# big-nacho/patolette

Hardware: AMD Instinct MI355X
Metric: Mpixels/sec quantized (256-color ICtCp + KMeans) at 1 GPU; palette ΔE vs ref (higher is better)
Workload: dtype f64

## Files before the change

patolette_amd/csrc/kmeans.hip:

```cpp
#include "kmeans.h"

namespace pamd {

typedef __attribute__((address_space(1))) const void gvoid_t;
typedef __attribute__((address_space(3))) void lvoid_t;

template <bool W>
__global__ __launch_bounds__(256) void k_km_gather(const double *__restrict__ planar, size_t N, const int *__restrict__ perm,
                                                   size_t nx, KmSamples s) {
    const size_t stride = (size_t)gridDim.x * blockDim.x;
    for (size_t i = (size_t)blockIdx.x * blockDim.x + threadIdx.x; i < nx; i += stride) {
        size_t p = perm ? (size_t)perm[i] : i;
        s.x[i] = (float)planar[p]; s.y[i] = (float)planar[N + p]; s.z[i] = (float)planar[2 * N + p];
        if constexpr (W) s.w[i] = (float)planar[3 * N + p];
    }
}

template <bool W>
__global__ __launch_bounds__(256) void k_km_gather_slice(const double *__restrict__ planar, size_t n_local, const int *__restrict__ perm,
                                                         size_t nx, size_t begin, KmSamples s) {
    const size_t stride = (size_t)gridDim.x * blockDim.x;
    for (size_t i = (size_t)blockIdx.x * blockDim.x + threadIdx.x; i < nx; i += stride) {
        const size_t g = perm ? (size_t)perm[i] : i;
        const bool mine = g >= begin && g - begin < n_local;
// ... 1184 lines not shown
    }
    return acc;
}

template <bool W, int C>
__device__ __forceinline__ float km_chain(const float4 *__restrict__ sorted, size_t lo, size_t hi, float4 (*stage)[64], int lane) {
    return km_chain_over<W, C>([=](const size_t i) { return sorted[lo + i]; }, hi - lo, stage, lane, 0.f);
}

template <int CTRL>
__device__ __forceinline__ double dpp_f64(const double v) {
    const unsigned long long b = (unsigned long long)__double_as_longlong(v);
    const int lo = __builtin_amdgcn_update_dpp(0, (int)(unsigned)b, CTRL, 0xf, 0xf, true);
    const int hi = __builtin_amdgcn_update_dpp(0, (int)(unsigned)(b >> 32), CTRL, 0xf, 0xf, true);
    return __longlong_as_double((long long)(((unsigned long long)(unsigned)hi << 32) | (unsigned)lo));
}
__device__ __forceinline__ double readlane_f64(const double v, const int l) {
    const unsigned long long b = (unsigned long long)__double_as_longlong(v);
    const unsigned lo = (unsigned)__builtin_amdgcn_readlane((int)(unsigned)b, l), hi = (unsigned)__builtin_amdgcn_readlane((int)(unsigned)(b >> 32), l);
    return __longlong_as_double((long long)(((unsigned long long)hi << 32) | lo));
}
__device__ __forceinline__ double wave_sum_dpp(double v) {
    v += dpp_f64<0xB1>(v);
    v += dpp_f64<0x4E>(v);
    v += dpp_f64<0x141>(v);
    v += dpp_f64<0x140>(v);
    return (readlane_f64(v, 0) + readlane_f64(v, 16)) + (readlane_f64(v, 32) + readlane_f64(v, 48));
}

__device__ __forceinline__ bool km_block_exact(const float *blk, const float *wblk, const bool wx, const int q0, const int nq, float &acc, const int lane) {
    const float aa = fabsf(acc);
    if (!(aa >= 1e-30f && aa < 1e30f)) return false;
    int ex;
    (void)frexpf(aa, &ex);
    const double sgn = acc < 0.f ? -1.0 : 1.0;
    const double scale = ldexp(sgn, 24 - ex);
    const double M0 = (double)aa * fabs(scale);
    double tot = 0.0, mag = 0.0, dev = 0.0;
    for (int q = q0; q < q0 + nq; q++) {
        const float4 xv = *reinterpret_cast<const float4 *>(blk + q * 256 + lane * 4);
        float4 wv = make_float4(1.f, 1.f, 1.f, 1.f);
        if (wx) wv = *reinterpret_cast<const float4 *>(wblk + q * 256 + lane * 4);
        const float xs[4] = {xv.x, xv.y, xv.z, xv.w}, ws[4] = {wv.x, wv.y, wv.z, wv.w};
#pragma unroll
        for (int e = 0; e < 4; e++) {
            const double x = (double)xs[e] * (double)ws[e];
            const double t = x * scale;
            const double r = rint(t);
            dev = fmax(dev, fabs(t - r));
            tot += r; mag += fabs(r);
        }
    }
    tot = wave_sum_dpp(tot); mag = wave_sum_dpp(mag);
    const double pp = 0.5 * (tot + mag), nn = 0.5 * (tot - mag);
    if (!__any(dev >= 0.5) && M0 + nn >= 8388609.0 && M0 + pp <= 16777215.0) {
        acc = (float)(ldexp(M0 + tot, ex - 24) * sgn);
        return true;
    }
    return false;
}
__device__ __forceinline__ void km_block_replay(const float *blk, const float *wblk, const bool wx, const unsigned from, const unsigned to, float &acc) {
    for (unsigned base = from; base < to; base += 64) {
        const int cnt = (int)(to - base < 64 ? to - base : 64);
        const float4 *s4 = reinterpret_cast<const float4 *>(blk + base), *w4 = reinterpret_cast<const float4 *>(wblk + base);
        if (cnt == 64) {
            float4 xv[16], wv[16];
#pragma unroll
            for (int q = 0; q < 16; q++) { xv[q] = s4[q]; if (wx) wv[q] = w4[q]; }
            if (wx) {
#pragma unroll
                for (int q = 0; q < 16; q++) {
                    acc = __builtin_fmaf(xv[q].x, wv[q].x, acc); acc = __builtin_fmaf(xv[q].y, wv[q].y, acc);
                    acc = __builtin_fmaf(xv[q].z, wv[q].z, acc); acc = __builtin_fmaf(xv[q].w, wv[q].w, acc);
                }
            } else {
#pragma unroll
                for (int q = 0; q < 16; q++) { acc += xv[q].x; acc += xv[q].y; acc += xv[q].z; acc += xv[q].w; }
            }
        } else {
            for (int q = 0; 4 * q < cnt; q++) {
                const float4 x = s4[q];
                float4 w = make_float4(0, 0, 0, 0);
                if (wx) w = w4[q];
                const float xs[4] = {x.x, x.y, x.z, x.w}, ws[4] = {w.x, w.y, w.z, w.w};
#pragma unroll
                for (int e = 0; e < 4; e++) {
                    if (4 * q + e < cnt) {
                        if (wx) acc = __builtin_fmaf(xs[e], ws[e], acc);
                        else acc += xs[e];
                    }
                }
            }
        }
    }
}
__device__ __forceinline__ void km_block_step(const float *blk, const float *wblk, const bool wx, const unsigned len, float &acc, const int lane) {
    if (km_block_exact(blk, wblk, wx, 0, 4, acc, lane)) return;
    if (len == 1024u) {
        for (int q = 0; q < 4; q++)
            if (!km_block_exact(blk, wblk, wx, q, 1, acc, lane)) km_block_replay(blk, wblk, wx, (unsigned)q * 256u, (unsigned)(q + 1) * 256u, acc);
        return;
    }
    km_block_replay(blk, wblk, wx, 0u, len, acc);
}

template <bool W>
__device__ __forceinline__ float km_chain_coop(const float4 *__restrict__ sorted, size_t lo, size_t hi, float *coop, int lane, int wid) {
    constexpr int K = 16;
    constexpr size_t BS = (size_t)64 * K, SS = 4 * BS;
    const bool wx = W && wid < 3;
    const bool chain = W || wid < 3;
    const float *mine = coop + (size_t)wid * SS, *wts = coop + 3 * SS;
    float acc = 0.f;
    float4 reg[K];
    auto fetch = [&](const size_t p0) {
#pragma unroll
        for (int j = 0; j < K; j++) {
            const size_t i = p0 + (size_t)wid * BS + (size_t)j * 64 + lane;
            reg[j] = make_float4(0, 0, 0, 0);
            if (i < hi) reg[j] = sorted[i];
        }
    };
    fetch(lo);
    for (size_t p0 = lo; p0 < hi; p0 += SS) {
#pragma unroll
        for (int j = 0; j < K; j++) {
            const int o = wid * (int)BS + j * 64 + lane;
            coop[o] = reg[j].x; coop[SS + o] = reg[j].y; coop[2 * SS + o] = reg[j].z; coop[3 * SS + o] = reg[j].w;
        }
        if (p0 + SS < hi) fetch(p0 + SS);
        __syncthreads();
        if (chain) {
            for (int d = 0; d < 4; d++) {
                const size_t pos = p0 + (size_t)d * BS;
                if (pos >= hi) break;
                const size_t bend = pos + BS < hi ? pos + BS : hi;
                const float *blk = mine + d * (int)BS, *wblk = wts + d * (int)BS;
                km_block_step(blk, wblk, wx, (unsigned)(bend - pos), acc, lane);
            }
        }
        __syncthreads();
    }
    return acc;
}

template <bool W>
__device__ __forceinline__ float km_coop_lds(const float *mine, const float *wts, const unsigned n, const bool wx, float acc, const int lane) {
    constexpr unsigned BS = 1024;
    for (unsigned pos = 0; pos < n; pos += BS)
        km_block_step(mine + pos, wts + pos, wx, pos + BS < n ? BS : n - pos, acc, lane);
    return acc;
}

template <bool W, int HS>
__device__ __forceinline__ void km_update_finish(const int kidx, const int k, const unsigned long long nx, const size_t cnt, const float *res,
                                                 int *s_last, float *cent, float *hassign, float4 *c4, unsigned int *ticket, DevMT *mt,
                                                 float *hs_mem = nullptr, unsigned int *flags = nullptr, const bool clean = false) {
    const int lane = threadIdx.x & 63, wid = threadIdx.x >> 6;
    float c0 = res[0], c1 = res[1], c2 = res[2], h = res[3];
    if constexpr (!W) {
        h = cnt < (size_t)16777216 ? (float)cnt : 16777216.0f;
    }
    if (threadIdx.x == 0) {
        if (!clean) {
        if (h != 0.f) { const float norm = 1 / h; c0 *= norm; c1 *= norm; c2 *= norm; }
        __hip_atomic_store(&cent[3 * kidx], c0, __ATOMIC_RELAXED, __HIP_MEMORY_SCOPE_AGENT);
        __hip_atomic_store(&cent[3 * kidx + 1], c1, __ATOMIC_RELAXED, __HIP_MEMORY_SCOPE_AGENT);
        __hip_atomic_store(&cent[3 * kidx + 2], c2, __ATOMIC_RELAXED, __HIP_MEMORY_SCOPE_AGENT);
        __hip_atomic_store(&hassign[kidx], h, __ATOMIC_RELAXED, __HIP_MEMORY_SCOPE_AGENT);
        km_store_c4(c4, k, kidx, c0, c1, c2);
        }
        asm volatile("s_waitcnt vmcnt(0)" ::: "memory");
        const unsigned tk = __hip_atomic_fetch_add(ticket, 1u, __ATOMIC_RELAXED, __HIP_MEMORY_SCOPE_AGENT);
        *s_last = (tk == (unsigned)k - 1u) ? 1 : 0;
    }
    __syncthreads();
    if (!*s_last || wid != 0) return;
    bool mine_empty = false, mine_dirty = false;
    for (int cb = 0; cb < k; cb += 256) {
        float hv[4]; unsigned fv[4];
#pragma unroll
        for (int q = 0; q < 4; q++) {
            const int ci = cb + 64 * q + lane;
            hv[q] = 1.f; fv[q] = 0u;
            if (ci < k) {
                hv[q] = __hip_atomic_load(&hassign[ci], __ATOMIC_RELAXED, __HIP_MEMORY_SCOPE_AGENT);
                if (flags) fv[q] = __hip_atomic_load(&flags[1 + ci], __ATOMIC_RELAXED, __HIP_MEMORY_SCOPE_AGENT);
            }
        }
#pragma unroll
        for (int q = 0; q < 4; q++) {
            const int ci = cb + 64 * q + lane;
            mine_empty = mine_empty || hv[q] == 0.f;
            mine_dirty = mine_dirty || fv[q] != 0u;
            if (flags && ci < k) __hip_atomic_store(&flags[1 + ci], 0u, __ATOMIC_RELAXED, __HIP_MEMORY_SCOPE_AGENT);
        }
    }
    const bool any = __ballot(mine_empty) != 0ULL;
    if (lane == 0) __hip_atomic_store(ticket, 0u, __ATOMIC_RELAXED, __HIP_MEMORY_SCOPE_AGENT);
    if (flags) {
        const bool any_dirty = __ballot(mine_dirty) != 0ULL;
        if (!any_dirty && !any && lane == 0) __hip_atomic_store(&flags[0], 1u, __ATOMIC_RELAXED, __HIP_MEMORY_SCOPE_AGENT);
    }
    if (!any) return;
    {
        asm volatile("s_waitcnt vmcnt(0)" ::: "memory");
        __shared__ unsigned s_mt[624];
        __builtin_amdgcn_fence(__ATOMIC_ACQUIRE, "agent");
        if constexpr (HS > 0) {
            __shared__ float s_hs[HS];
            km_split_clusters_wave<false>(cent, hassign, k, nx, mt, s_mt, s_hs, lane, flags);
        } else km_split_clusters_wave<true>(cent, hassign, k, nx, mt, s_mt, hs_mem, lane);
        __builtin_amdgcn_fence(__ATOMIC_RELEASE, "agent");
        asm volatile("s_waitcnt vmcnt(0)" ::: "memory");
    }
    for (int j = lane; j < k; j += 64) {
        const float v0 = __hip_atomic_load(&cent[3 * j], __ATOMIC_RELAXED, __HIP_MEMORY_SCOPE_AGENT);
        const float v1 = __hip_atomic_load(&cent[3 * j + 1], __ATOMIC_RELAXED, __HIP_MEMORY_SCOPE_AGENT);
        const float v2 = __hip_atomic_load(&cent[3 * j + 2], __ATOMIC_RELAXED, __HIP_MEMORY_SCOPE_AGENT);
        km_store_c4(c4, k, j, v0, v1, v2);
    }
}

template <bool W, bool BIGK = false>
__global__ __launch_bounds__(256) void k_km_update(const float4 *__restrict__ sorted, const unsigned int *__restrict__ rowtot, int k,
                                                  unsigned long long nx, float *cent, float *hassign, float4 *c4,
                                                  unsigned int *ticket, DevMT *mt, unsigned long long long_min, float *hs_mem) {
    __shared__ float4 stage[4][2][64];
    extern __shared__ __attribute__((aligned(16))) float coop[];
    __shared__ float res[4];
    __shared__ int s_last;
    const int kidx = blockIdx.x, lane = threadIdx.x & 63, wid = threadIdx.x >> 6;
    unsigned pre = 0;
    for (int j = lane; j < kidx; j += 64) pre += rowtot[j];
    pre = wave_sum_u32(pre);
    pre = __shfl(pre, 0, 64);
    const size_t lo = pre, hi = lo + rowtot[kidx];
    float acc = 0.f;
    if ((size_t)(hi - lo) >= long_min) {
        acc = km_chain_coop<W>(sorted, lo, hi, coop, lane, wid);
    } else {
        if (wid == 0) acc = km_chain<W, 0>(sorted, lo, hi, stage[0], lane);
        else if (wid == 1) acc = km_chain<W, 1>(sorted, lo, hi, stage[1], lane);
        else if (wid == 2) acc = km_chain<W, 2>(sorted, lo, hi, stage[2], lane);
        else if (W) acc = km_chain<W, 3>(sorted, lo, hi, stage[3], lane);
    }
    if (lane == 0) res[wid] = acc;
    __syncthreads();
    km_update_finish<W, BIGK ? 0 : kKMeansMaxK>(kidx, k, nx, hi - lo, res, &s_last, cent, hassign, c4, ticket, mt, hs_mem);
}

constexpr int kKmDirectCap = 4096;
constexpr int kKmSortBlock = 1024;

__device__ __forceinline__ unsigned block_scan_incl_u32(const unsigned v, unsigned *wsum, unsigned *total) {
    const int lane = threadIdx.x & 63, wid = threadIdx.x >> 6, nw = (int)(blockDim.x >> 6);
    const unsigned inc = wave_scan_incl_u32(v);
    __syncthreads();
    if (lane == 63) wsum[wid] = inc;
    __syncthreads();
    unsigned pre = 0, all = 0;
    for (int w = 0; w < nw; w++) { const unsigned t = wsum[w]; all += t; pre += w < wid ? t : 0u; }
    *total = all;
    return pre + inc;
}

typedef float f2_t __attribute__((ext_vector_type(2)));
typedef float f8_t __attribute__((ext_vector_type(8)));
typedef const __attribute__((address_space(4))) f8_t *scalar_c8_t;

__device__ __forceinline__ float km_min3(const float a, const float b, const float c) {
    float r;
    asm("v_min3_f32 %0, %1, %2, %3" : "=v"(r) : "v"(a), "v"(b), "v"(c));
    return r;
}
__device__ __forceinline__ int km_assign_min3(const float x0, const float x1, const float x2, const scalar_c4_t c4,
                                              const scalar_c8_t c8, const float4 *c4s, const int k) {
    const f2_t m0 = {-2 * x0, -2 * x0}, m1 = {-2 * x1, -2 * x1}, m2 = {-2 * x2, -2 * x2};
    const float xn = __builtin_fmaf(x2, x2, __builtin_fmaf(x0, x0, x1 * x1));
    float ld[8]; int lc[8];
#pragma unroll
    for (int l = 0; l < 8; l++) { ld[l] = 3.402823466e+38F - xn; lc[l] = -1; }
    const int ny_p = (k / 8) * 8;
    const int U = ny_p >> 4;
    const int CUN = (U + 3) >> 2;
    auto pair_dp = [&](const f8_t y) {
        const f2_t y0 = {y[0], y[1]}, y1 = {y[2], y[3]}, y2 = {y[4], y[5]}, yw = {y[6], y[7]};
        f2_t dp = m0 * y0;
        dp = __builtin_elementwise_fma(m1, y1, dp);
        dp = __builtin_elementwise_fma(m2, y2, dp);
        return dp + yw;
    };
    for (int c = 0; c < 4; c++) {
        const int u0 = c * CUN, u1 = u0 + CUN < U ? u0 + CUN : U;
        if (u0 >= u1) break;
        float snap[8];
#pragma unroll
        for (int l = 0; l < 8; l++) snap[l] = ld[l];
        for (int u = u0; u < u1; u++) {
            const int p0 = u << 3;
            typedef float f16_t __attribute__((ext_vector_type(16)));
            typedef const __attribute__((address_space(4))) f16_t *scalar_c16_t;
            const scalar_c16_t c16 = (scalar_c16_t)c8;
            const f16_t q0 = c16[p0 >> 1], q1 = c16[(p0 >> 1) + 1], q2 = c16[(p0 >> 1) + 2], q3 = c16[(p0 >> 1) + 3];
            auto half = [](const f16_t q, const int h) { return h ? f8_t{q[8], q[9], q[10], q[11], q[12], q[13], q[14], q[15]} : f8_t{q[0], q[1], q[2], q[3], q[4], q[5], q[6], q[7]}; };
#pragma unroll
            for (int l = 0; l < 8; l += 2) {
                const f8_t ya = half(l < 4 ? q0 : q1, (l >> 1) & 1), yb = half(l < 4 ? q2 : q3, (l >> 1) & 1);
                const f2_t a = pair_dp(ya), b = pair_dp(yb);
                ld[l] = km_min3(ld[l], a[0], b[0]);
                ld[l + 1] = km_min3(ld[l + 1], a[1], b[1]);
            }
        }
#pragma unroll
        for (int l = 0; l < 8; l++) lc[l] = ld[l] < snap[l] ? c : lc[l];
    }
    if (ny_p & 8) {
        const int p0 = U << 3;
#pragma unroll
        for (int l = 0; l < 8; l += 2) {
            const f2_t a = pair_dp(c8[p0 + (l >> 1)]);
            if (a[0] < ld[l]) { ld[l] = a[0]; lc[l] = 4; }
            if (a[1] < ld[l + 1]) { ld[l + 1] = a[1]; lc[l + 1] = 4; }
        }
    }
    float cand[8];
    float cur_d = 3.402823466e+38F;
#pragma unroll
    for (int l = 0; l < 8; l++) { float cd = ld[l] + xn; if (cd < 0) cd = 0; cand[l] = cd; cur_d = cd < cur_d ? cd : cur_d; }
    unsigned tm = 0u;
#pragma unroll
    for (int l = 0; l < 8; l++) tm |= cand[l] == cur_d ? (1u << l) : 0u;
    unsigned cur_i = 0xFFFFFFFFu;
    while (__any(tm != 0u)) {
        if (tm) {
            const int l = __ffs((int)tm) - 1;
            tm &= tm - 1u;
            float target = ld[0]; int c = lc[0];
#pragma unroll
            for (int q = 1; q < 8; q++) { target = l == q ? ld[q] : target; c = l == q ? lc[q] : c; }
            unsigned idx = 0u;
            if (c == 4) idx = (unsigned)((U << 4) + l);
            else if (c >= 0) {
                const int u0 = c * CUN, u1 = u0 + CUN < U ? u0 + CUN : U;
                const int base = (u0 << 4) + l, lim = u1 << 4;
                for (int q = 2 * CUN - 1; q >= 0; q--) {
                    const int j = base + 8 * q;
                    if (j < lim) {
                        const float4 y = c4s[j];
                        float dp = (-2 * x0) * y.x;
                        dp = __builtin_fmaf(-2 * x1, y.y, dp);
                        dp = __builtin_fmaf(-2 * x2, y.z, dp);
                        dp = dp + y.w;
                        if (dp == target) idx = (unsigned)j;
                    }
                }
            }
            cur_i = idx < cur_i ? idx : cur_i;
        }
    }
    for (int j0 = ny_p; j0 < k; j0++) {
        const auto y = c4[j0];
        float dp = __builtin_fmaf(x2, y.z, __builtin_fmaf(x1, y.y, x0 * y.x));
        float d = xn + y.w - 2 * dp;
        if (d < 0) d = 0;
        if (cur_d > d) { cur_d = d; cur_i = (unsigned)j0; }
    }
    return cur_i < (unsigned)k ? (int)cur_i : 0;
}

#ifdef PAMD_KM_TRACE
__device__ unsigned long long g_km_trace[2][256][32];
#define KM_TRACE(kern, slot) do { if ((threadIdx.x & 63) == 0) g_km_trace[kern][blockIdx.x & 255][slot] = wall_clock64(); } while (0)
#define KM_TRACE0(kern, slot) do { if (threadIdx.x == 0) g_km_trace[kern][blockIdx.x & 255][slot] = wall_clock64(); } while (0)
#else
#define KM_TRACE(kern, slot) do { } while (0)
#define KM_TRACE0(kern, slot) do { } while (0)
#endif

__global__ __launch_bounds__(1024) void k_km_assign_sort(KmSamples s, size_t nx, const float4 *__restrict__ c4, int k, const bool weighted,
                                                         float4 *__restrict__ sorted_rec, unsigned short *__restrict__ offs,
                                                         unsigned char *__restrict__ prev, unsigned int *flags) {
    if (flags[0]) return;
    __shared__ unsigned char cnt[16][256];
    __shared__ unsigned short stepbase[16][256];
    __shared__ unsigned int wsum[16];
    __shared__ float4 c4s[256];
    const int lane = threadIdx.x & 63, step = threadIdx.x >> 6;
    KM_TRACE0(0, 0);
    for (int i = threadIdx.x; i < 16 * 256 / 4; i += 1024) reinterpret_cast<unsigned int *>(&cnt[0][0])[i] = 0u;
    if ((int)threadIdx.x < k) c4s[threadIdx.x] = c4[threadIdx.x];
    __syncthreads();
    KM_TRACE0(0, 1);
    const scalar_c4_t t4 = (scalar_c4_t)(unsigned long long)c4;
    const scalar_c8_t t8 = (scalar_c8_t)(unsigned long long)(c4 + k);
    const size_t blk0 = (size_t)blockIdx.x * kKmSortBlock;
    const size_t i = blk0 + (size_t)step * 64 + lane;
    const bool v = i < nx;
    float4 rec = make_float4(0.f, 0.f, 0.f, 0.f);
    if (v) { rec.x = s.x[i]; rec.y = s.y[i]; rec.z = s.z[i]; if (weighted) rec.w = s.w[i]; }
#ifdef PAMD_KM_TRACE
    asm volatile("s_waitcnt vmcnt(0)" ::: "memory");
    KM_TRACE0(0, 2);
    if (threadIdx.x == 0) g_km_trace[0][blockIdx.x & 255][24] = clock64();
#endif
    int a = km_assign_min3(rec.x, rec.y, rec.z, t4, t8, c4s, k);
    if (!v) a = 0;
    if (v) {
        const int old = prev[i];
        if (old != a) { prev[i] = (unsigned char)a; flags[1 + old] = 1u; flags[1 + a] = 1u; }
    }
    const unsigned long long m = match_mask(a, 8, __ballot(v));
    const unsigned rk = (unsigned)__popcll(m & ((1ULL << lane) - 1ULL));
    if (v && rk == 0u) cnt[step][a] = (unsigned char)__popcll(m);
#ifdef PAMD_KM_TRACE
    if (lane == 0) g_km_trace[0][blockIdx.x & 255][8 + step] = wall_clock64();
    if (threadIdx.x == 0) g_km_trace[0][blockIdx.x & 255][25] = clock64();
#endif
    __syncthreads();
    KM_TRACE0(0, 3);
    unsigned tot = 0;
    unsigned short pre[16];
    if (threadIdx.x < 256) {
#pragma unroll
        for (int st = 0; st < 16; st++) { pre[st] = (unsigned short)tot; tot += cnt[st][threadIdx.x]; }
    }
    unsigned total = 0;
    const unsigned start = block_scan_incl_u32(tot, wsum, &total) - tot;
    if (threadIdx.x < 256) {
#pragma unroll
        for (int st = 0; st < 16; st++) stepbase[st][threadIdx.x] = (unsigned short)(start + pre[st]);
        unsigned short *ob = offs + (size_t)blockIdx.x * 257;
        ob[threadIdx.x] = (unsigned short)start;
        if (threadIdx.x == 255) ob[256] = (unsigned short)total;
    }
    __syncthreads();
    KM_TRACE0(0, 4);
    if (v) sorted_rec[blk0 + (unsigned)stepbase[step][a] + rk] = rec;
#ifdef PAMD_KM_TRACE
    asm volatile("s_waitcnt vmcnt(0)" ::: "memory");
    KM_TRACE0(0, 5);
#endif
}

template <bool W>
__global__ __launch_bounds__(256) void k_km_update_lists(const float4 *__restrict__ sorted_rec, const unsigned short *__restrict__ offs,
                                                        unsigned long long nx, int k, float *cent, float *hassign, float4 *c4,
                                                        unsigned int *ticket, DevMT *mt, unsigned int *flags) {
    if (flags[0]) return;
    __shared__ float4 stage[4][2][64];
    extern __shared__ __attribute__((aligned(16))) float members[];
    __shared__ float res[4];
    __shared__ int s_last;
    __shared__ unsigned int wsum[16];
    __shared__ unsigned int n_long, long_src[256], long_lo[256], long_nb[256];
    const int kidx = blockIdx.x, lane = threadIdx.x & 63, wid = threadIdx.x >> 6;
    float *const mx = members, *const my = members + kKmDirectCap, *const mz = members + 2 * kKmDirectCap, *const mw = members + 3 * kKmDirectCap;
    unsigned int *const srcidx = reinterpret_cast<unsigned int *>(members + 4 * kKmDirectCap);
    float acc = 0.f;
    size_t total = 0;
    unsigned fill = 0;
    KM_TRACE0(1, 0);
    bool long_list = false;
    auto replay = [&]() {
        const unsigned n = fill;
        if (n == (unsigned)kKmDirectCap || long_list) {
            const unsigned padded = (n + 1023u) & ~1023u;
            for (unsigned i = n + threadIdx.x; i < padded; i += 256) { mx[i] = 0.f; my[i] = 0.f; mz[i] = 0.f; mw[i] = 0.f; }
            __syncthreads();
            if ((W || wid < 3) && n) acc = km_coop_lds<W>(members + (size_t)wid * kKmDirectCap, mw, n, W && wid < 3, acc, lane);
            long_list = true;
            return;
        }
        auto rec = [&](const size_t i) { return make_float4(mx[i], my[i], mz[i], mw[i]); };
        if (wid == 0) acc = km_chain_over<W, 0>(rec, n, stage[0], lane, acc);
        else if (wid == 1) acc = km_chain_over<W, 1>(rec, n, stage[1], lane, acc);
        else if (wid == 2) acc = km_chain_over<W, 2>(rec, n, stage[2], lane, acc);
        else if (W) acc = km_chain_over<W, 3>(rec, n, stage[3], lane, acc);
    };
    const bool clean = flags[1 + kidx] == 0u;
    const unsigned long long nblocks = clean ? 0ULL : (nx + kKmSortBlock - 1) / kKmSortBlock;
    for (unsigned long long c0 = 0; c0 < nblocks; c0 += 256) {
        const unsigned long long b = c0 + threadIdx.x;
        unsigned o0 = 0, nb = 0;
        if (b < nblocks) { o0 = offs[b * 257 + kidx]; nb = (unsigned)offs[b * 257 + kidx + 1] - o0; }
        unsigned chunk_total = 0;
        const unsigned excl = block_scan_incl_u32(nb, wsum, &chunk_total) - nb;
        constexpr unsigned kLongRun = 32;
        const bool is_long = nb > kLongRun;
        if (threadIdx.x == 0) n_long = 0u;
        __syncthreads();
        if (is_long) { const unsigned e = atomicAdd(&n_long, 1u); long_src[e] = (unsigned)(b * kKmSortBlock) + o0; long_lo[e] = excl; long_nb[e] = nb; }
        __syncthreads();
        const unsigned nl = n_long;
        unsigned done = 0;
        while (done < chunk_total) {
            const unsigned take = min((unsigned)kKmDirectCap - fill, chunk_total - done);
            if (!is_long) {
                const unsigned lo = max(excl, done), hi = min(excl + nb, done + take);
                const float4 *src = sorted_rec + b * kKmSortBlock + o0;
                for (unsigned q = lo; q < hi; q += 4) {
                    float4 r4[4];
#pragma unroll
                    for (int u = 0; u < 4; u++) r4[u] = q + u < hi ? src[q + u - excl] : make_float4(0.f, 0.f, 0.f, 0.f);
#pragma unroll
                    for (int u = 0; u < 4; u++) if (q + u < hi) { const unsigned i = fill + q + u - done; mx[i] = r4[u].x; my[i] = r4[u].y; mz[i] = r4[u].z; mw[i] = r4[u].w; }
                }
            }
            if (nl) {
                for (unsigned i = threadIdx.x; i < take; i += 256) srcidx[fill + i] = ~0u;
                __syncthreads();
                for (unsigned e = 0; e < nl; e++) {
                    const unsigned ex0 = long_lo[e], lo = max(ex0, done), hi = min(ex0 + long_nb[e], done + take);
                    for (unsigned q = lo + threadIdx.x; q < hi; q += 256) srcidx[fill + q - done] = long_src[e] + (q - ex0);
                }
                __syncthreads();
                for (unsigned i0 = threadIdx.x; i0 < take; i0 += 256 * 8) {
                    unsigned ix[8]; float4 r[8];
#pragma unroll
                    for (int u = 0; u < 8; u++) { const unsigned i = i0 + 256u * u; ix[u] = i < take ? srcidx[fill + i] : ~0u; }
#pragma unroll
                    for (int u = 0; u < 8; u++) r[u] = ix[u] != ~0u ? sorted_rec[ix[u]] : make_float4(0.f, 0.f, 0.f, 0.f);
#pragma unroll
                    for (int u = 0; u < 8; u++) if (ix[u] != ~0u) { const unsigned i = fill + i0 + 256u * u; mx[i] = r[u].x; my[i] = r[u].y; mz[i] = r[u].z; mw[i] = r[u].w; }
                }
            }
            fill += take; done += take;
            __syncthreads();
            if (fill == (unsigned)kKmDirectCap) { replay(); fill = 0; __syncthreads(); }
        }
        total += chunk_total;
    }
    __syncthreads();
    KM_TRACE0(1, 1);
    replay();
#ifdef PAMD_KM_TRACE
    if (lane == 0) g_km_trace[1][blockIdx.x & 255][8 + wid] = wall_clock64();
#endif
    if (lane == 0) res[wid] = acc;
    __syncthreads();
    KM_TRACE0(1, 2);
    km_update_finish<W, 256>(kidx, k, nx, total, res, &s_last, cent, hassign, c4, ticket, mt, nullptr, flags, clean);
    KM_TRACE0(1, 3);
}

struct KmFix { double magic_x, quantum_x, magic_w, quantum_w; };
__device__ __forceinline__ long long km_fix_quant(const double v, const double magic) {
    return __double_as_longlong(v + magic) - __double_as_longlong(magic);
}
template <bool W, typename AT>
__global__ __launch_bounds__(256) void k_km_accum(KmSamples s, const AT *__restrict__ assign, size_t nx, int k, KmFix f,
                                                  unsigned long long *gsum ) {
    extern __shared__ unsigned long long acc64[];
    for (int i = threadIdx.x; i < 4 * k; i += 256) acc64[i] = 0ULL;
    __syncthreads();
    auto add = [&](const unsigned a, const float x, const float y, const float z, const float w) {
        const double wd = W ? (double)w : 1.0;
        unsigned long long *r = acc64 + 4 * (size_t)a;
        atomicAdd(r, (unsigned long long)km_fix_quant((double)x * wd, f.magic_x));
        atomicAdd(r + 1, (unsigned long long)km_fix_quant((double)y * wd, f.magic_x));
        atomicAdd(r + 2, (unsigned long long)km_fix_quant((double)z * wd, f.magic_x));
        atomicAdd(r + 3, W ? (unsigned long long)km_fix_quant(wd, f.magic_w) : 1ULL);
    };
    const size_t stride = (size_t)gridDim.x * 1024;
    for (size_t base = ((size_t)blockIdx.x * 256 + threadIdx.x) * 4; base < nx; base += stride) {
        if (base + 4 <= nx) {
            const float4 vx = *reinterpret_cast<const float4 *>(s.x + base), vy = *reinterpret_cast<const float4 *>(s.y + base),
                         vz = *reinterpret_cast<const float4 *>(s.z + base);
            float4 vw = make_float4(1.f, 1.f, 1.f, 1.f);
            if constexpr (W) vw = *reinterpret_cast<const float4 *>(s.w + base);
            unsigned a0, a1, a2, a3;
            if constexpr (sizeof(AT) == 1) {
                const unsigned pk = *reinterpret_cast<const unsigned int *>(assign + base);
                a0 = pk & 0xffu; a1 = (pk >> 8) & 0xffu; a2 = (pk >> 16) & 0xffu; a3 = pk >> 24;
            } else {
                const int4 pk = *reinterpret_cast<const int4 *>(assign + base);
                a0 = (unsigned)pk.x; a1 = (unsigned)pk.y; a2 = (unsigned)pk.z; a3 = (unsigned)pk.w;
            }
            add(a0, vx.x, vy.x, vz.x, vw.x); add(a1, vx.y, vy.y, vz.y, vw.y);
            add(a2, vx.z, vy.z, vz.z, vw.z); add(a3, vx.w, vy.w, vz.w, vw.w);
        } else {
            for (size_t i = base; i < nx; i++) add((unsigned)assign[i], s.x[i], s.y[i], s.z[i], W ? s.w[i] : 1.f);
        }
    }
    __syncthreads();
    for (int i = threadIdx.x; i < 4 * k; i += 256) { const unsigned long long v = acc64[i]; if (v) atomicAdd(&gsum[i], v); }
}

template <bool W>
__global__ __launch_bounds__(256) void k_km_update_sums(unsigned long long *gsum, int k, unsigned long long nx, KmFix f, float *cent,
                                                        float *hassign, float4 *c4, DevMT *mt) {
    __shared__ int s_empty;
    if (threadIdx.x == 0) s_empty = 0;
    __syncthreads();
    for (int j = threadIdx.x; j < k; j += 256) {
        const double sx = (double)(long long)gsum[4 * j] * f.quantum_x, sy = (double)(long long)gsum[4 * j + 1] * f.quantum_x,
                     sz = (double)(long long)gsum[4 * j + 2] * f.quantum_x;
        float h;
        if constexpr (W) h = (float)((double)(long long)gsum[4 * j + 3] * f.quantum_w);
        else h = (float)gsum[4 * j + 3];
        float c0 = (float)sx, c1 = (float)sy, c2 = (float)sz;
        if (h != 0.f) { const float norm = 1 / h; c0 *= norm; c1 *= norm; c2 *= norm; }
        else s_empty = 1;
        cent[3 * j] = c0; cent[3 * j + 1] = c1; cent[3 * j + 2] = c2; hassign[j] = h;
        gsum[4 * j] = 0ULL; gsum[4 * j + 1] = 0ULL; gsum[4 * j + 2] = 0ULL; gsum[4 * j + 3] = 0ULL;
    }
    __threadfence();
    __syncthreads();
    if (s_empty && threadIdx.x < 64) {
        __shared__ unsigned s_mt[624];
        __shared__ float s_hs[kKMeansMaxK];
        km_split_clusters_wave(cent, hassign, k, nx, mt, s_mt, s_hs, (int)threadIdx.x);
        __threadfence();
    }
    __syncthreads();
    for (int j = threadIdx.x; j < k; j += 256) km_store_c4(c4, k, j, cent[3 * j], cent[3 * j + 1], cent[3 * j + 2]);
}

static int chunk_len_for(size_t nx) {
    size_t c = ceil_div(nx, 4096);
    c = ceil_div(c, 64) * 64;
    if (c < 64) c = 64;
    return (int)c;
}

void KMeansWork::reserve(size_t nx, int k) {
    sx.reserve(nx); sy.reserve(nx); sz.reserve(nx); sw.reserve(nx);
    assign.reserve(nx); sorted.reserve(nx);
    const int nchunks = (int)ceil_div(nx, (size_t)chunk_len_for(nx));
    table.reserve(std::max((size_t)k * (size_t)(nchunks > 0 ? nchunks : 1),
                           (ceil_div(nx, (size_t)1024) * 257 + 1) / 2 + 1));
    rowtot.reserve(k);
    if (k > kKMeansMaxK) { rowbase.reserve(k); hs.reserve(k); }
    cent.reserve(3 * (size_t)k); hassign.reserve(k); c4.reserve(2 * (size_t)k + 2);
    perm.reserve(nx);
    if (!mt.p) { mt.reserve(1); mt_seeded = false; }
    if (!ticket.p) { ticket.reserve(1); HIP_CHECK(hipMemset(ticket.p, 0, sizeof(unsigned int))); }
    flags.reserve(2 + 256);
}

void kmeans_gather(const double *d_planar, size_t N, bool weighted, const int *d_perm, size_t nx, KMeansWork &w, hipStream_t s) {
    KmSamples ks{w.sx.p, w.sy.p, w.sz.p, w.sw.p};
    size_t g = ceil_div(nx, 256);
    if (g > 4096) g = 4096;
    if (g < 1) g = 1;
    KTIME("k_km_gather", s, (weighted ? 48.0 : 36.0) * nx);
    if (weighted) hipLaunchKernelGGL(k_km_gather<true>, (int)g, 256, 0, s, d_planar, N, d_perm, nx, ks);
    else hipLaunchKernelGGL(k_km_gather<false>, (int)g, 256, 0, s, d_planar, N, d_perm, nx, ks);
    HIP_CHECK(hipGetLastError());
}

void kmeans_gather_slice(const double *d_planar, size_t n_local, bool weighted, const int *d_perm, size_t nx, size_t begin,
                         KMeansWork &w, hipStream_t s) {
    KmSamples ks{w.sx.p, w.sy.p, w.sz.p, w.sw.p};
    size_t g = ceil_div(nx, 256);
    if (g > 4096) g = 4096;
    if (g < 1) g = 1;
    KTIME("k_km_gather", s, (weighted ? 48.0 : 36.0) * nx);
    if (weighted) hipLaunchKernelGGL(k_km_gather_slice<true>, (int)g, 256, 0, s, d_planar, n_local, d_perm, nx, begin, ks);
    else hipLaunchKernelGGL(k_km_gather_slice<false>, (int)g, 256, 0, s, d_planar, n_local, d_perm, nx, begin, ks);
    HIP_CHECK(hipGetLastError());
}

void kmeans_iterate(KMeansWork &w, size_t nx, int k, bool weighted, int niter, hipStream_t s, size_t expect_longest, const KmSums *sums) {
    KmSamples ks{w.sx.p, w.sy.p, w.sz.p, w.sw.p};
    KmFix fix{};
    int ablocks = 1;
    if (sums && k > kKMeansMaxK) sums = nullptr;
    if (sums) {
        int ex = 0, ew = 0, P = 1;
        (void)frexp(std::max(sums->bound_x, 1e-300) * (weighted ? std::max(sums->bound_w, 1e-300) : 1.0), &ex);
        (void)frexp(std::max(sums->bound_w, 1e-300), &ew);
        while (((size_t)1 << P) < nx) P++;
        P = std::max(P + 1, 12);
        fix.quantum_x = ldexp(1.0, ex + P - 62); fix.magic_x = ldexp(1.5, 52 + ex + P - 62);
        fix.quantum_w = ldexp(1.0, ew + P - 62); fix.magic_w = ldexp(1.5, 52 + ew + P - 62);
        w.fsum.reserve(4 * (size_t)k);
        HIP_CHECK(hipMemsetAsync(w.fsum.p, 0, 4 * (size_t)k * sizeof(unsigned long long), s));
        ablocks = (int)std::min<size_t>(std::max<size_t>(ceil_div(nx, (size_t)4096), 1), 2048);
        static PerDeviceOnce attr5;
        attr5.once([&] {
            HIP_CHECK(hipFuncSetAttribute((const void *)k_km_accum<true, int>, hipFuncAttributeMaxDynamicSharedMemorySize, 32 * kKMeansMaxK));
            HIP_CHECK(hipFuncSetAttribute((const void *)k_km_accum<false, int>, hipFuncAttributeMaxDynamicSharedMemorySize, 32 * kKMeansMaxK));
            HIP_CHECK(hipFuncSetAttribute((const void *)k_km_accum<true, unsigned char>, hipFuncAttributeMaxDynamicSharedMemorySize, 32 * kKMeansMaxK));
            HIP_CHECK(hipFuncSetAttribute((const void *)k_km_accum<false, unsigned char>, hipFuncAttributeMaxDynamicSharedMemorySize, 32 * kKMeansMaxK));
        });
    }
    auto update_sums = [&](const bool a8) {
        {
            KTIME("k_km_accum", s, ((weighted ? 16.0 : 12.0) + (a8 ? 1.0 : 4.0)) * nx);
            const size_t lds = (size_t)32 * k;
            if (a8) {
                if (weighted) hipLaunchKernelGGL((k_km_accum<true, unsigned char>), ablocks, 256, lds, s, ks, (const unsigned char *)w.assign.p, nx, k, fix, w.fsum.p);
                else hipLaunchKernelGGL((k_km_accum<false, unsigned char>), ablocks, 256, lds, s, ks, (const unsigned char *)w.assign.p, nx, k, fix, w.fsum.p);
            } else {
// ... 180 lines not shown
```

Measured before the change: 3075.

## Fold dirty/empty status into ticket counter and hoist loads before early exit

The ticket atomic now carries packed dirty and empty counts, so the last-arriving block knows whether any cluster is empty or dirty without rescanning hassign and the per-cluster flags. Each block clears its own dirty flag when it finishes. In the assign-sort and update-lists kernels, the sample, prev, centroid and offs loads are issued before the converged-flag check, so global-memory latency overlaps with that check. This removes a serial scan over k clusters at the end of each iteration and shortens kernel startup latency. In exchange, blocks do redundant loads even when converged, and correctness now depends on the packed counter fields not overflowing for k up to 256.

Result: no change. 3088, median of 6 (+0.4%).

```diff
diff --git a/patolette_amd/csrc/kmeans.hip b/patolette_amd/csrc/kmeans.hip
--- a/patolette_amd/csrc/kmeans.hip
+++ b/patolette_amd/csrc/kmeans.hip
@@ -1360,10 +1360,12 @@
     return acc;
 }
 
+constexpr unsigned kKmTicketDirty = 1u << 10, kKmTicketEmpty = 1u << 20, kKmTicketField = (1u << 10) - 1u;
 template <bool W, int HS>
 __device__ __forceinline__ void km_update_finish(const int kidx, const int k, const unsigned long long nx, const size_t cnt, const float *res,
                                                  int *s_last, float *cent, float *hassign, float4 *c4, unsigned int *ticket, DevMT *mt,
-                                                 float *hs_mem = nullptr, unsigned int *flags = nullptr, const bool clean = false) {
+                                                 float *hs_mem = nullptr, unsigned int *flags = nullptr, const bool clean = false,
+                                                 const float h_stands = 1.f) {
     const int lane = threadIdx.x & 63, wid = threadIdx.x >> 6;
     float c0 = res[0], c1 = res[1], c2 = res[2], h = res[3];
     if constexpr (!W) {
@@ -1377,38 +1379,44 @@
         __hip_atomic_store(&cent[3 * kidx + 2], c2, __ATOMIC_RELAXED, __HIP_MEMORY_SCOPE_AGENT);
         __hip_atomic_store(&hassign[kidx], h, __ATOMIC_RELAXED, __HIP_MEMORY_SCOPE_AGENT);
         km_store_c4(c4, k, kidx, c0, c1, c2);
+        if (flags) __hip_atomic_store(&flags[1 + kidx], 0u, __ATOMIC_RELAXED, __HIP_MEMORY_SCOPE_AGENT);
         }
         asm volatile("s_waitcnt vmcnt(0)" ::: "memory");
-        const unsigned tk = __hip_atomic_fetch_add(ticket, 1u, __ATOMIC_RELAXED, __HIP_MEMORY_SCOPE_AGENT);
-        *s_last = (tk == (unsigned)k - 1u) ? 1 : 0;
+        if (flags) {
+            const unsigned add = 1u + (clean ? 0u : kKmTicketDirty) + ((clean ? h_stands : h) == 0.f ? kKmTicketEmpty : 0u);
+            const unsigned all = __hip_atomic_fetch_add(ticket, add, __ATOMIC_RELAXED, __HIP_MEMORY_SCOPE_AGENT) + add;
+            const bool last = (all & kKmTicketField) == (unsigned)k;
+            *s_last = !last ? 0 : 1 | ((all >> 20) & kKmTicketField ? 2 : 0) | ((all >> 10) & kKmTicketField ? 4 : 0);
+        } else {
+            const unsigned tk = __hip_atomic_fetch_add(ticket, 1u, __ATOMIC_RELAXED, __HIP_MEMORY_SCOPE_AGENT);
+            *s_last = (tk == (unsigned)k - 1u) ? 1 : 0;
+        }
     }
     __syncthreads();
     if (!*s_last || wid != 0) return;
-    bool mine_empty = false, mine_dirty = false;
+    bool any;
+    if (flags) {
+        any = (*s_last & 2) != 0;
+        const bool any_dirty = (*s_last & 4) != 0;
+        if (lane == 0) {
+            __hip_atomic_store(ticket, 0u, __ATOMIC_RELAXED, __HIP_MEMORY_SCOPE_AGENT);
+            if (!any_dirty && !any) __hip_atomic_store(&flags[0], 1u, __ATOMIC_RELAXED, __HIP_MEMORY_SCOPE_AGENT);
+        }
+    } else {
+    bool mine_empty = false;
     for (int cb = 0; cb < k; cb += 256) {
-        float hv[4]; unsigned fv[4];
+        float hv[4];
 #pragma unroll
         for (int q = 0; q < 4; q++) {
             const int ci = cb + 64 * q + lane;
-            hv[q] = 1.f; fv[q] = 0u;
-            if (ci < k) {
-                hv[q] = __hip_atomic_load(&hassign[ci], __ATOMIC_RELAXED, __HIP_MEMORY_SCOPE_AGENT);
-                if (flags) fv[q] = __hip_atomic_load(&flags[1 + ci], __ATOMIC_RELAXED, __HIP_MEMORY_SCOPE_AGENT);
-            }
-        }
-#pragma unroll
-        for (int q = 0; q < 4; q++) {
-            const int ci = cb + 64 * q + lane;
-            mine_empty = mine_empty || hv[q] == 0.f;
-            mine_dirty = mine_dirty || fv[q] != 0u;
-            if (flags && ci < k) __hip_atomic_store(&flags[1 + ci], 0u, __ATOMIC_RELAXED, __HIP_MEMORY_SCOPE_AGENT);
-        }
-    }
-    const bool any = __ballot(mine_empty) != 0ULL;
+            hv[q] = 1.f;
+            if (ci < k) hv[q] = __hip_atomic_load(&hassign[ci], __ATOMIC_RELAXED, __HIP_MEMORY_SCOPE_AGENT);
+        }
+#pragma unroll
+        for (int q = 0; q < 4; q++) mine_empty = mine_empty || hv[q] == 0.f;
+    }
+    any = __ballot(mine_empty) != 0ULL;
     if (lane == 0) __hip_atomic_store(ticket, 0u, __ATOMIC_RELAXED, __HIP_MEMORY_SCOPE_AGENT);
-    if (flags) {
-        const bool any_dirty = __ballot(mine_dirty) != 0ULL;
-        if (!any_dirty && !any && lane == 0) __hip_atomic_store(&flags[0], 1u, __ATOMIC_RELAXED, __HIP_MEMORY_SCOPE_AGENT);
     }
     if (!any) return;
     {
@@ -1589,24 +1597,28 @@
 __global__ __launch_bounds__(1024) void k_km_assign_sort(KmSamples s, size_t nx, const float4 *__restrict__ c4, int k, const bool weighted,
                                                          float4 *__restrict__ sorted_rec, unsigned short *__restrict__ offs,
                                                          unsigned char *__restrict__ prev, unsigned int *flags) {
-    if (flags[0]) return;
     __shared__ unsigned char cnt[16][256];
     __shared__ unsigned short stepbase[16][256];
     __shared__ unsigned int wsum[16];
     __shared__ float4 c4s[256];
     const int lane = threadIdx.x & 63, step = threadIdx.x >> 6;
     KM_TRACE0(0, 0);
-    for (int i = threadIdx.x; i < 16 * 256 / 4; i += 1024) reinterpret_cast<unsigned int *>(&cnt[0][0])[i] = 0u;
-    if ((int)threadIdx.x < k) c4s[threadIdx.x] = c4[threadIdx.x];
-    __syncthreads();
-    KM_TRACE0(0, 1);
-    const scalar_c4_t t4 = (scalar_c4_t)(unsigned long long)c4;
-    const scalar_c8_t t8 = (scalar_c8_t)(unsigned long long)(c4 + k);
     const size_t blk0 = (size_t)blockIdx.x * kKmSortBlock;
     const size_t i = blk0 + (size_t)step * 64 + lane;
     const bool v = i < nx;
     float4 rec = make_float4(0.f, 0.f, 0.f, 0.f);
-    if (v) { rec.x = s.x[i]; rec.y = s.y[i]; rec.z = s.z[i]; if (weighted) rec.w = s.w[i]; }
+    int old = 0;
+    if (v) { rec.x = s.x[i]; rec.y = s.y[i]; rec.z = s.z[i]; if (weighted) rec.w = s.w[i]; old = prev[i]; }
+    const unsigned fixed = flags[0];
+    float4 trow = make_float4(0.f, 0.f, 0.f, 0.f);
+    if ((int)threadIdx.x < k) trow = c4[threadIdx.x];
+    for (int z = threadIdx.x; z < 16 * 256 / 4; z += 1024) reinterpret_cast<unsigned int *>(&cnt[0][0])[z] = 0u;
+    if ((int)threadIdx.x < k) c4s[threadIdx.x] = trow;
+    __syncthreads();
+    if (fixed) return;
+    KM_TRACE0(0, 1);
+    const scalar_c4_t t4 = (scalar_c4_t)(unsigned long long)c4;
+    const scalar_c8_t t8 = (scalar_c8_t)(unsigned long long)(c4 + k);
 #ifdef PAMD_KM_TRACE
     asm volatile("s_waitcnt vmcnt(0)" ::: "memory");
     KM_TRACE0(0, 2);
@@ -1615,7 +1627,6 @@
     int a = km_assign_min3(rec.x, rec.y, rec.z, t4, t8, c4s, k);
     if (!v) a = 0;
     if (v) {
-        const int old = prev[i];
         if (old != a) { prev[i] = (unsigned char)a; flags[1 + old] = 1u; flags[1 + a] = 1u; }
     }
     const unsigned long long m = match_mask(a, 8, __ballot(v));
@@ -1655,7 +1666,6 @@
 __global__ __launch_bounds__(256) void k_km_update_lists(const float4 *__restrict__ sorted_rec, const unsigned short *__restrict__ offs,
                                                         unsigned long long nx, int k, float *cent, float *hassign, float4 *c4,
                                                         unsigned int *ticket, DevMT *mt, unsigned int *flags) {
-    if (flags[0]) return;
     __shared__ float4 stage[4][2][64];
     extern __shared__ __attribute__((aligned(16))) float members[];
     __shared__ float res[4];
@@ -1686,12 +1696,26 @@
         else if (wid == 2) acc = km_chain_over<W, 2>(rec, n, stage[2], lane, acc);
         else if (W) acc = km_chain_over<W, 3>(rec, n, stage[3], lane, acc);
     };
-    const bool clean = flags[1 + kidx] == 0u;
-    const unsigned long long nblocks = clean ? 0ULL : (nx + kKmSortBlock - 1) / kKmSortBlock;
+    const unsigned long long nblocks_all = (nx + kKmSortBlock - 1) / kKmSortBlock;
+    const size_t b_first = threadIdx.x < nblocks_all ? (size_t)threadIdx.x : (size_t)(nblocks_all - 1);
+    unsigned o0_first = __hip_atomic_load(&offs[b_first * 257 + kidx], __ATOMIC_RELAXED, __HIP_MEMORY_SCOPE_AGENT);
+    unsigned o1_first = __hip_atomic_load(&offs[b_first * 257 + kidx + 1], __ATOMIC_RELAXED, __HIP_MEMORY_SCOPE_AGENT);
+    const unsigned fixed = __hip_atomic_load(&flags[0], __ATOMIC_RELAXED, __HIP_MEMORY_SCOPE_AGENT);
+    const unsigned dirty = __hip_atomic_load(&flags[1 + kidx], __ATOMIC_RELAXED, __HIP_MEMORY_SCOPE_AGENT);
+    const float h_stands = __hip_atomic_load(&hassign[kidx], __ATOMIC_RELAXED, __HIP_MEMORY_SCOPE_AGENT);
+    if (fixed) return;
+    if (threadIdx.x >= nblocks_all) o0_first = o1_first = 0u;
+    const bool clean = dirty == 0u;
+    const unsigned long long nblocks = clean ? 0ULL : nblocks_all;
+#ifdef PAMD_KM_TRACE
+    asm volatile("s_waitcnt vmcnt(0)" ::: "memory");
+    KM_TRACE0(1, 6);
+#endif
     for (unsigned long long c0 = 0; c0 < nblocks; c0 += 256) {
         const unsigned long long b = c0 + threadIdx.x;
         unsigned o0 = 0, nb = 0;
-        if (b < nblocks) { o0 = offs[b * 257 + kidx]; nb = (unsigned)offs[b * 257 + kidx + 1] - o0; }
+        if (c0 == 0) { o0 = o0_first; nb = o1_first - o0_first; }
+        else if (b < nblocks) { o0 = offs[b * 257 + kidx]; nb = (unsigned)offs[b * 257 + kidx + 1] - o0; }
         unsigned chunk_total = 0;
         const unsigned excl = block_scan_incl_u32(nb, wsum, &chunk_total) - nb;
         constexpr unsigned kLongRun = 32;
@@ -1748,7 +1772,10 @@
     if (lane == 0) res[wid] = acc;
     __syncthreads();
     KM_TRACE0(1, 2);
-    km_update_finish<W, 256>(kidx, k, nx, total, res, &s_last, cent, hassign, c4, ticket, mt, nullptr, flags, clean);
+#ifdef PAMD_KM_TRACE
+    if (threadIdx.x == 0) { g_km_trace[1][blockIdx.x & 255][4] = total; g_km_trace[1][blockIdx.x & 255][5] = clean ? 1ULL : 0ULL; }
+#endif
+    km_update_finish<W, 256>(kidx, k, nx, total, res, &s_last, cent, hassign, c4, ticket, mt, nullptr, flags, clean, h_stands);
     KM_TRACE0(1, 3);
 }
 
```
